# althonos/pyhmmer

Measured on AMD Instinct MI355X. Metric: GCUPS (DP cells/s) + seqs/s for hmmsearch, Pfam-A vs proteome, 1/2/4/8 GPUs, higher is better.
Workload: dtype u8/i16 filters (MSV, Viterbi), f32 Forward/Backward

## Files before the change

### pyhmmer_amd/csrc/p7x_vitpk.hip

```cpp
#include "p7x_wave.hpp"
#include "p7x_launch.hpp"

namespace p7x {

namespace {

typedef short s2v __attribute__((ext_vector_type(2)));
__device__ __forceinline__ s2v as_s2v(uint32_t u) { return __builtin_bit_cast(s2v, u); }
__device__ __forceinline__ uint32_t as_u(s2v v) { return __builtin_bit_cast(uint32_t, v); }
__device__ __forceinline__ uint32_t pk_adds(uint32_t a, uint32_t b) { return as_u(__builtin_elementwise_add_sat(as_s2v(a), as_s2v(b))); }
__device__ __forceinline__ uint32_t pk_max(uint32_t a, uint32_t b) { return as_u(__builtin_elementwise_max(as_s2v(a), as_s2v(b))); }
__device__ __forceinline__ uint32_t splat16(int v) { const uint32_t w = (uint32_t) v & 0xffffu; return w | (w << 16); }
__device__ __forceinline__ int lo_of(uint32_t w) { return (int) (short) (w & 0xffffu); }
__device__ __forceinline__ int hi_of(uint32_t w) { return (int) (short) (w >> 16); }

constexpr uint32_t kNeg2 = 0x80008000u;
constexpr int vitpk_rowq(int T, int P)
{
  const int n = ((P + 3) / 4) * T;
  return T == 8 ? ((n & 15) == 8 ? n : n + 8) : n;
}

#define P7X_DPP_U(v, ctrl) ((uint32_t) __builtin_amdgcn_update_dpp((int) kNeg2, (int) (v), (ctrl), 0xf, 0xf, false))

template <int T>
__device__ __forceinline__ int group_max(uint32_t v)
{
  v = pk_max(v, P7X_DPP_U(v, 0xB1));
  v = pk_max(v, P7X_DPP_U(v, 0x4E));
  v = pk_max(v, P7X_DPP_U(v, 0x141));
  if constexpr (T >= 16) v = pk_max(v, P7X_DPP_U(v, 0x140));
  if constexpr (T >= 32) {
    const auto x = __builtin_amdgcn_permlane16_swap(v, v, false, false);
    v = pk_max(x[0], x[1]);
  }
  if constexpr (T == 64) {
    const auto x = __builtin_amdgcn_permlane32_swap(v, v, false, false);
    v = pk_max(x[0], x[1]);
  }
  return max(lo_of(v), hi_of(v));
}

}

struct RowState { int xN, xB, xJ, xC; bool overflow; };

template <int T>
__device__ __forceinline__ uint32_t stripe_shift(uint32_t r, bool first, bool hi)
{
  if constexpr (T == 64) {
    const uint32_t w = P7X_DPP_U(r, 0x13C);
    return first ? ((w << 16) | 0x8000u) : w;
  }
  const uint32_t prev = P7X_DPP_U(r, 0x138);
  uint32_t last;
  if constexpr (T == 32) {
    const uint32_t l31 = (uint32_t) __builtin_amdgcn_readlane((int) r, 31), l63 = (uint32_t) __builtin_amdgcn_readlane((int) r, 63);
    last = hi ? l63 : l31;
  } else last = P7X_DPP_U(r, T == 8 ? 0x141 : 0x140);
  return first ? ((last << 16) | 0x8000u) : prev;
}

template <int T, int P>
__device__ __forceinline__ void vit_row(const VitPkArgs &a, const uint4 *tral, const uint4 *trbl, const uint4 *er, bool first, bool hi,
                                        bool active, int xwm, const uint32_t (&mi)[P], const uint32_t (&ii)[P],
                                        const uint32_t (&di)[P], uint32_t (&mo_)[P], uint32_t (&io_)[P], uint32_t (&do_)[P],
                                        const uint32_t (&tdd)[P], RowState &rs)
{
  constexpr int PS = (P + 3) & ~3;
  const uint32_t xBv = splat16(rs.xB);
  uint32_t mp = stripe_shift<T>(mi[P - 1], first, hi), ip = stripe_shift<T>(ii[P - 1], first, hi), dp = stripe_shift<T>(di[P - 1], first, hi);
  uint32_t xEv = kNeg2, dmaxv = kNeg2, dcv = kNeg2;
#pragma unroll
  for (int j4 = 0; j4 < PS; j4 += 4) {
    const uint4 e4 = er[(j4 / 4) * T];
    const uint32_t ev[4] = { e4.x, e4.y, e4.z, e4.w };
#pragma unroll
    for (int jj = 0; jj < 4; ++jj) {
      const int q = j4 + jj;
      if (q < P) {
        const uint4 ta = tral[q * T], tb = trbl[q * T];
        const uint32_t a0 = pk_adds(xBv, ta.x), a1 = pk_adds(mp, ta.y), a2 = pk_adds(ip, ta.z), a3 = pk_adds(dp, ta.w);
        uint32_t sv = pk_max(pk_max(a0, a1), pk_max(a2, a3));
        sv = pk_adds(sv, ev[jj]);
        xEv = pk_max(xEv, sv);
        mo_[q] = sv;
        if (q > 0) do_[q] = dcv;
        dcv = pk_adds(sv, tb.x);
        dmaxv = pk_max(dmaxv, dcv);
        io_[q] = pk_max(pk_adds(mi[q], tb.y), pk_adds(ii[q], tb.z));
        mp = mi[q]; ip = ii[q]; dp = di[q];
      }
    }
    asm volatile("" ::: "memory");
  }
  do_[0] = stripe_shift<T>(dcv, first, hi);
  const int xE = group_max<T>(xEv);
  const int Dmax = group_max<T>(dmaxv);
  if (active) {
    if (xE >= 32767) rs.overflow = true;
    rs.xC = max(rs.xC, xE + a.xw_e);
    rs.xJ = max(rs.xJ, xE + a.xw_e);
    rs.xB = max(rs.xJ + xwm, rs.xN + xwm);
  }
  const bool trig = active && (Dmax + a.ddbound > rs.xB);
#ifdef P7X_VITPK_NO_CLOSURE
  if (false) {
#else
  if (__any(trig)) {
#endif
    int pass = 0;
    bool more;
    do {
#pragma unroll
      for (int q = 1; q < P; ++q) do_[q] = pk_max(do_[q], pk_adds(do_[q - 1], tdd[q - 1]));
      uint32_t c = stripe_shift<T>(pk_adds(do_[P - 1], tdd[P - 1]), first, hi);
      if (!trig) c = kNeg2;
      const uint32_t d0 = pk_max(do_[0], c);
      const bool changed = d0 != do_[0];
      do_[0] = d0;
      more = __any(changed) && ++pass < 2 * T;
    } while (more);
  }
}

constexpr int vitpk_waves(int T, int P)
{
  if (T == 64) return P <= 12 ? 16 : 12;
  if (T == 32) return (P >= 13 && P <= 16) ? 12 : 8;
  return 4;
}

template <int T, int P>
__global__ void __launch_bounds__(64 * vitpk_waves(T, P)) vitpk_kernel(const ArgRef ref)
{
  constexpr int G = 64 / T;
  constexpr int NW = vitpk_waves(T, P), NT = 64 * NW;
  const VitPkArgs a = load_args<VitPkArgs>(ref);
  const int nlist = a.nlist_ptr ? *a.nlist_ptr : a.nlist;
  const int nskip = a.nskip_ptr ? *a.nskip_ptr : 0;
  if (nskip + (int) (blockIdx.x * NW * G) >= nlist) return;
  constexpr int PS = (P + 3) & ~3;
  constexpr int ROWQ = vitpk_rowq(T, P);
  extern __shared__ __attribute__((aligned(16))) unsigned char smem[];
  uint4 *tra = reinterpret_cast<uint4 *>(smem);
  uint4 *trb = tra + P * T;
  uint4 *em = trb + P * T;
  {
    const uint4 *gt = reinterpret_cast<const uint4 *>(a.trans);
    for (int i = threadIdx.x; i < 2 * P * T; i += NT) tra[i] = gt[i];
    const uint4 *ge = reinterpret_cast<const uint4 *>(a.emis);
    for (int i = threadIdx.x; i < a.nrows * ROWQ; i += NT) em[i] = ge[i];
  }
  __syncthreads();
  const int lane = threadIdx.x & 63;
  const int s = lane % T, g = lane / T;
  const bool first = (s == 0), hi = (g != 0);
  const int wave0 = rfl((int) (blockIdx.x * NW + (threadIdx.x >> 6)));
  const int nwaves = (int) gridDim.x * NW;
  const uint4 *tral = tra + s, *trbl = trb + s, *eml = em + s;
  uint32_t tdd[P];
#pragma unroll
  for (int q = 0; q < P; ++q) tdd[q] = trbl[q * T].w;

  for (int it0 = nskip + wave0 * G; it0 < nlist; it0 += nwaves * G) {
    const int it = it0 + g;
    const bool have = it < nlist;
    const int slot = have ? (a.list ? a.list[it] : it) : 0;
    const int L = have ? a.slot_len[slot] : 0;
    const uint8_t *sq = a.dsq + (have ? a.slot_off[slot] : 0);
    const int xwm = (int) a.xwmove_tab[L];
    const int Lmax = wave_max_i32(L);

    uint32_t mA[P], iA[P], dA[P], mB[P], iB[P], dB[P];
#pragma unroll
    for (int j = 0; j < P; ++j) mA[j] = iA[j] = dA[j] = kNeg2;
    RowState rs;
    rs.xN = a.base_w; rs.xB = rs.xN + xwm; rs.xJ = -32768; rs.xC = -32768; rs.overflow = false;

    for (int i0 = 0; i0 < Lmax; i0 += 4 * T) {
      uint32_t word = 0;
#pragma unroll
      for (int b = 0; b < 4; ++b) {
        const int r = i0 + 4 * s + b;
        const uint32_t x = (r < L) ? (uint32_t) sq[r] : 0u;
        word |= x << (8 * b);
      }
      const int nrow = min(4 * T, Lmax - i0);
      auto residue = [&](int r) -> uint32_t {
        const uint32_t w = (uint32_t) __shfl((int) word, g * T + (r >> 2));
        return (w >> (8 * (r & 3))) & 0xffu;
      };
      int r = 0;
      for (; r + 1 < nrow; r += 2) {
        vit_row<T, P>(a, tral, trbl, eml + residue(r) * ROWQ, first, hi, i0 + r < L, xwm, mA, iA, dA, mB, iB, dB, tdd, rs);
        vit_row<T, P>(a, tral, trbl, eml + residue(r + 1) * ROWQ, first, hi, i0 + r + 1 < L, xwm, mB, iB, dB, mA, iA, dA, tdd, rs);
      }
      if (r < nrow) {
        vit_row<T, P>(a, tral, trbl, eml + residue(r) * ROWQ, first, hi, i0 + r < L, xwm, mA, iA, dA, mB, iB, dB, tdd, rs);
#pragma unroll
        for (int j = 0; j < P; ++j) { mA[j] = mB[j]; iA[j] = iB[j]; dA[j] = dB[j]; }
      }
    }
    const bool overflow = rs.overflow; const int xC = rs.xC;
    if (have && s == 0) a.out_xC[it] = overflow ? 32767 : xC;
  }
}

#define P7X_VITPK_TILES(X) \
  X(8, 2) X(8, 4) X(8, 6) X(8, 8) X(8, 10) X(8, 12) X(8, 14) X(8, 15) X(8, 16) X(8, 17) X(8, 18) X(8, 19) X(8, 20) \
  X(16, 11) X(16, 12) X(16, 13) X(16, 14) X(16, 15) X(16, 16) X(16, 17) X(16, 18) X(16, 19) X(16, 20) \
  X(32, 11) X(32, 12) X(32, 13) X(32, 14) X(32, 15) X(32, 16) X(32, 17) X(32, 18) X(32, 19) X(32, 20) \
  X(64, 11) X(64, 12) X(64, 13) X(64, 14) X(64, 15) X(64, 16)

bool vitpk_pick(int M, int *T, int *P)
{
  const bool wide = debug_opt(OPT_VIT_WIDE) != 0;
#define P7X_PK(TT, PP) if (M <= 2 * TT * PP) { if (TT >= 32 && !wide) return false; *T = TT; *P = PP; return true; }
  P7X_VITPK_TILES(P7X_PK)
#undef P7X_PK
  return false;
}

void vitpk_build_tables(const Profile &p, int T, int P, std::vector<uint32_t> &trans, std::vector<uint32_t> &emis)
{
  const int rowq = vitpk_rowq(T, P), nrows = p.Kp + 1;
  auto pack = [](int lo, int hi) { return ((uint32_t) lo & 0xffffu) | (((uint32_t) hi & 0xffffu) << 16); };
  trans.assign((size_t) 2 * P * T * 4, kNeg2);
  emis.assign((size_t) nrows * rowq * 4, kNeg2);
  for (int s = 0; s < T; ++s)
    for (int j = 0; j < P; ++j) {
      const int k0 = s * P + j + 1, k1 = (s + T) * P + j + 1;
      for (int t = 0; t < NTRANS; ++t) {
        const int lo = (k0 <= p.M) ? p.tw[(size_t) t * (p.M + 1) + k0] : -32768;
        const int hi = (k1 <= p.M) ? p.tw[(size_t) t * (p.M + 1) + k1] : -32768;
        trans[((size_t) (t / 4) * P * T + (size_t) j * T + s) * 4 + (t % 4)] = pack(lo, hi);
      }
      for (int x = 0; x < p.Kp; ++x) {
        const int lo = (k0 <= p.M) ? p.rw[(size_t) x * (p.M + 1) + k0] : -32768;
        const int hi = (k1 <= p.M) ? p.rw[(size_t) x * (p.M + 1) + k1] : -32768;
        emis[((size_t) x * rowq + (size_t) (j / 4) * T + s) * 4 + (j % 4)] = pack(lo, hi);
      }
    }
}

template <int T, int P>
static int launch_pk(const ArgRun<VitPkArgs> &a, int num_cu, hipStream_t st)
{
  const size_t lds = ((size_t) 2 * P * T + (size_t) a.at(0).nrows * vitpk_rowq(T, P)) * 16;
  auto kern = vitpk_kernel<T, P>;
  constexpr int NW = vitpk_waves(T, P), NT = 64 * NW;
  int per_cu = 0;
  const int pst = kernel_blocks_per_cu(kern, NT, lds, &per_cu);
  if (pst != P7X_OK) return pst;
  long want = 0;
  for (int i = 0; i < a.n; ++i) want = std::max<long>(want, ((long) a.at(i).nlist + NW * (64 / T) - 1) / (NW * (64 / T)));
  if (want <= 0) return P7X_OK;
  hipLaunchKernelGGL(kern, dim3(lane_grid(want, (long) num_cu * per_cu, a.n), (unsigned) a.n), dim3(NT), lds, st, a.ref());
  P7X_HIP(hipGetLastError());
  return P7X_OK;
}

int vitpk_launch(int T, int P, const ArgRun<VitPkArgs> &a, int num_cu, hipStream_t st)
{
  if (a.n <= 0) return P7X_OK;
#define P7X_PK(TT, PP) if (T == TT && P == PP) return launch_pk<TT, PP>(a, num_cu, st);
  P7X_VITPK_TILES(P7X_PK)
#undef P7X_PK
  set_error("no packed Viterbi kernel for this model length");
  return P7X_EINVAL;
}

}
```

Baseline: 26520.

## Fold one D-D step into the Viterbi row sweep and merge group reductions

The packed Viterbi row now applies one delete-to-delete step inline while computing D cells, so the lazy-F closure loop should trigger and iterate less often. The xE and Dmax cross-lane reductions are packed into a single DPP reduction, and the DPP fallback now uses bound_ctrl with zero instead of the negative sentinel. The tdd transition registers are loaded only inside the closure, which frees registers. The kernel also adds a minimum-waves hint to launch bounds and prefetches the next residue word one row pair ahead. Optional atomic row counters are added behind a compile flag for profiling. The risks are that the added launch-bounds hint could cause spills, and that the changed DPP fill value could alter results in lanes that read invalid neighbours.

```diff
diff --git a/pyhmmer_amd/csrc/p7x_vitpk.hip b/pyhmmer_amd/csrc/p7x_vitpk.hip
--- a/pyhmmer_amd/csrc/p7x_vitpk.hip
+++ b/pyhmmer_amd/csrc/p7x_vitpk.hip
@@ -21,11 +21,12 @@
   return T == 8 ? ((n & 15) == 8 ? n : n + 8) : n;
 }
 
-#define P7X_DPP_U(v, ctrl) ((uint32_t) __builtin_amdgcn_update_dpp((int) kNeg2, (int) (v), (ctrl), 0xf, 0xf, false))
+#define P7X_DPP_U(v, ctrl) ((uint32_t) __builtin_amdgcn_update_dpp(0, (int) (v), (ctrl), 0xf, 0xf, true))
 
 template <int T>
-__device__ __forceinline__ int group_max(uint32_t v)
-{
+__device__ __forceinline__ void group_max2(uint32_t a, uint32_t b, int &amax, int &bmax)
+{
+  uint32_t v = pk_max(__builtin_amdgcn_perm(b, a, 0x05040100u), __builtin_amdgcn_perm(b, a, 0x07060302u));
   v = pk_max(v, P7X_DPP_U(v, 0xB1));
   v = pk_max(v, P7X_DPP_U(v, 0x4E));
   v = pk_max(v, P7X_DPP_U(v, 0x141));
@@ -38,8 +39,12 @@
     const auto x = __builtin_amdgcn_permlane32_swap(v, v, false, false);
     v = pk_max(x[0], x[1]);
   }
-  return max(lo_of(v), hi_of(v));
-}
+  amax = lo_of(v); bmax = hi_of(v);
+}
+
+#ifdef P7X_VITPK_COUNT
+__device__ unsigned long long vitpk_row_counts[3];
+#endif
 
 }
 
@@ -65,12 +70,13 @@
 __device__ __forceinline__ void vit_row(const VitPkArgs &a, const uint4 *tral, const uint4 *trbl, const uint4 *er, bool first, bool hi,
                                         bool active, int xwm, const uint32_t (&mi)[P], const uint32_t (&ii)[P],
                                         const uint32_t (&di)[P], uint32_t (&mo_)[P], uint32_t (&io_)[P], uint32_t (&do_)[P],
-                                        const uint32_t (&tdd)[P], RowState &rs)
+                                        RowState &rs)
 {
   constexpr int PS = (P + 3) & ~3;
   const uint32_t xBv = splat16(rs.xB);
   uint32_t mp = stripe_shift<T>(mi[P - 1], first, hi), ip = stripe_shift<T>(ii[P - 1], first, hi), dp = stripe_shift<T>(di[P - 1], first, hi);
   uint32_t xEv = kNeg2, dmaxv = kNeg2, dcv = kNeg2;
+  uint32_t ddp = kNeg2;
 #pragma unroll
   for (int j4 = 0; j4 < PS; j4 += 4) {
     const uint4 e4 = er[(j4 / 4) * T];
@@ -85,7 +91,9 @@
         sv = pk_adds(sv, ev[jj]);
         xEv = pk_max(xEv, sv);
         mo_[q] = sv;
-        if (q > 0) do_[q] = dcv;
+        if (q == 1) do_[1] = dcv;
+        if (q > 1) do_[q] = pk_max(dcv, pk_adds(do_[q - 1], ddp));
+        ddp = tb.w;
         dcv = pk_adds(sv, tb.x);
         dmaxv = pk_max(dmaxv, dcv);
         io_[q] = pk_max(pk_adds(mi[q], tb.y), pk_adds(ii[q], tb.z));
@@ -94,9 +102,9 @@
     }
     asm volatile("" ::: "memory");
   }
-  do_[0] = stripe_shift<T>(dcv, first, hi);
-  const int xE = group_max<T>(xEv);
-  const int Dmax = group_max<T>(dmaxv);
+  do_[0] = stripe_shift<T>(pk_max(dcv, pk_adds(do_[P - 1], ddp)), first, hi);
+  int xE, Dmax;
+  group_max2<T>(xEv, dmaxv, xE, Dmax);
   if (active) {
     if (xE >= 32767) rs.overflow = true;
     rs.xC = max(rs.xC, xE + a.xw_e);
@@ -104,11 +112,21 @@
     rs.xB = max(rs.xJ + xwm, rs.xN + xwm);
   }
   const bool trig = active && (Dmax + a.ddbound > rs.xB);
+#ifdef P7X_VITPK_COUNT
+  const bool count_lane = (threadIdx.x & 63) == 0;
+  if (count_lane) atomicAdd(&vitpk_row_counts[0], 1ull);
+#endif
 #ifdef P7X_VITPK_NO_CLOSURE
   if (false) {
 #else
   if (__any(trig)) {
 #endif
+#ifdef P7X_VITPK_COUNT
+    if (count_lane) atomicAdd(&vitpk_row_counts[1], 1ull);
+#endif
+    uint32_t tdd[P];
+#pragma unroll
+    for (int q = 0; q < P; ++q) tdd[q] = trbl[q * T].w;
     int pass = 0;
     bool more;
     do {
@@ -120,6 +138,9 @@
       const bool changed = d0 != do_[0];
       do_[0] = d0;
       more = __any(changed) && ++pass < 2 * T;
+#ifdef P7X_VITPK_COUNT
+      if (count_lane) atomicAdd(&vitpk_row_counts[2], 1ull);
+#endif
     } while (more);
   }
 }
@@ -131,8 +152,15 @@
   return 4;
 }
 
+constexpr int vitpk_simd_waves(int T, int P)
+{
+  if (T == 64) return P <= 12 ? 4 : 3;
+  if (T == 32) return P <= 12 ? 4 : P <= 16 ? 3 : 2;
+  return P <= 2 ? 8 : P <= 4 ? 7 : P <= 6 ? 6 : P <= 8 ? 5 : P <= 12 ? 4 : P <= 17 ? 3 : 2;
+}
+
 template <int T, int P>
-__global__ void __launch_bounds__(64 * vitpk_waves(T, P)) vitpk_kernel(const ArgRef ref)
+__global__ void __launch_bounds__(64 * vitpk_waves(T, P), vitpk_simd_waves(T, P)) vitpk_kernel(const ArgRef ref)
 {
   constexpr int G = 64 / T;
   constexpr int NW = vitpk_waves(T, P), NT = 64 * NW;
@@ -159,10 +187,6 @@
   const int wave0 = rfl((int) (blockIdx.x * NW + (threadIdx.x >> 6)));
   const int nwaves = (int) gridDim.x * NW;
   const uint4 *tral = tra + s, *trbl = trb + s, *eml = em + s;
-  uint32_t tdd[P];
-#pragma unroll
-  for (int q = 0; q < P; ++q) tdd[q] = trbl[q * T].w;
-
   for (int it0 = nskip + wave0 * G; it0 < nlist; it0 += nwaves * G) {
     const int it = it0 + g;
     const bool have = it < nlist;
@@ -187,17 +211,18 @@
         word |= x << (8 * b);
       }
       const int nrow = min(4 * T, Lmax - i0);
-      auto residue = [&](int r) -> uint32_t {
-        const uint32_t w = (uint32_t) __shfl((int) word, g * T + (r >> 2));
-        return (w >> (8 * (r & 3))) & 0xffu;
-      };
+      auto fetch = [&](int r) -> uint32_t { return (uint32_t) __shfl((int) word, g * T + min(r >> 2, T - 1)); };
+      auto residue = [](uint32_t w, int r) -> uint32_t { return (w >> (8 * (r & 3))) & 0xffu; };
+      uint32_t w = fetch(0);
       int r = 0;
       for (; r + 1 < nrow; r += 2) {
-        vit_row<T, P>(a, tral, trbl, eml + residue(r) * ROWQ, first, hi, i0 + r < L, xwm, mA, iA, dA, mB, iB, dB, tdd, rs);
-        vit_row<T, P>(a, tral, trbl, eml + residue(r + 1) * ROWQ, first, hi, i0 + r + 1 < L, xwm, mB, iB, dB, mA, iA, dA, tdd, rs);
+        const uint32_t wn = fetch(r + 2);
+        vit_row<T, P>(a, tral, trbl, eml + residue(w, r) * ROWQ, first, hi, i0 + r < L, xwm, mA, iA, dA, mB, iB, dB, rs);
+        vit_row<T, P>(a, tral, trbl, eml + residue(w, r + 1) * ROWQ, first, hi, i0 + r + 1 < L, xwm, mB, iB, dB, mA, iA, dA, rs);
+        w = wn;
       }
       if (r < nrow) {
-        vit_row<T, P>(a, tral, trbl, eml + residue(r) * ROWQ, first, hi, i0 + r < L, xwm, mA, iA, dA, mB, iB, dB, tdd, rs);
+        vit_row<T, P>(a, tral, trbl, eml + residue(w, r) * ROWQ, first, hi, i0 + r < L, xwm, mA, iA, dA, mB, iB, dB, rs);
 #pragma unroll
         for (int j = 0; j < P; ++j) { mA[j] = mB[j]; iA[j] = iB[j]; dA[j] = dB[j]; }
       }
@@ -272,3 +297,11 @@
 }
 
 }
+
+#ifdef P7X_VITPK_COUNT
+extern "C" int p7x_vitpk_row_counts(unsigned long long *out)
+{
+  if (hipDeviceSynchronize() != hipSuccess) return -1;
+  return hipMemcpyFromSymbol(out, HIP_SYMBOL(p7x::vitpk_row_counts), 3 * sizeof(unsigned long long)) == hipSuccess ? 0 : -1;
+}
+#endif
```

Result: faster. 27150 (median of 6 runs) (+2.4%).
